# kendricktan/simple-zk-rollups

Hardware: AMD Instinct MI355X
Metric: Groth16 proofs/sec (rollup batch circuit) (higher is better)
Workload: dtype u32 limbs, 254-bit integer Montgomery (9 x 29 bits in the MSM kernels, 8 x 32 bits elsewhere); 1 GPU; 2^20-constraint synthetic rollup circuit, 1 proof per step per GPU; log_m=20, n_public=73, nVars=1048576, nnzA=1827887, nnzB=1577678, parallelism=proof-sharded x1 (key arena replicated once: single), proofs_in_flight=2

## Files before the change

include/zkr.h:

```cpp
#ifndef ZKR_H
#define ZKR_H
#include <stddef.h>
#include <stdint.h>

#ifdef __cplusplus
extern "C" {
#endif

typedef enum {
  ZKR_OK = 0,
  ZKR_ERR_NO_DEVICE = -1,
  ZKR_ERR_BAD_KEY = -2,
  ZKR_ERR_BAD_WITNESS = -3,
  ZKR_ERR_HIP = -4,
  ZKR_ERR_ARG = -5,
  ZKR_ERR_DEGENERATE = -6,
  ZKR_ERR_UNSATISFIED = -7
} zkr_status;

typedef struct zkr_key zkr_key;

const char *zkr_last_error(void);
const char *zkr_version(void);
int zkr_device_count(void);
// ... 220 lines not shown
int zkr_operator_new(zkr_ledger *l, zkr_key *key, zkr_r1cs *cs, zkr_vk *vk, const zkr_operator_opts *opts, zkr_operator **out);
void zkr_operator_free(zkr_operator *op);
int zkr_operator_info(const zkr_operator *op, uint64_t out[6]);
int zkr_operator_step(zkr_operator *op, const uint8_t *txs, size_t n_txs, const uint8_t *r32s, const uint8_t *s32s, uint8_t *status, uint8_t *proofs_out,
                      void *publics_out, size_t *n_batches, size_t *consumed);
int zkr_operator_stage_times(const zkr_operator *op, double ms[6]);

int zkr_selftest_f29_forms(int device, int field, int form, const uint32_t *records, size_t n, uint32_t *out);
int zkr_selftest_curve29(int device, int g2, int op, const uint32_t *records, size_t n, uint32_t *out, uint8_t *inf);
int zkr_selftest_fp(int device, int field, int op, const uint32_t *records, size_t n, uint32_t *out);
typedef struct {
  uint32_t logn, tlog, dif, inverse, pre, nbat, pair, in_place, want_lo, want_n, coset_shift, coset_add;
  uint32_t cross, klog, col_lo, col_n, in_sub, out_sub, canon, reserved;
} zkr_ntt_selftest_desc;
int zkr_selftest_ntt(int device, const zkr_ntt_selftest_desc *desc, void *in0, void *in1, void *out, void *in0_b, void *in1_b, void *out_b);
int zkr_bench_fq_mul(int device, double *gmuls_per_s);
int zkr_bench_fq_mul_legacy(int device, double *gmuls_per_s);

#ifdef __cplusplus
}
#endif
#endif
```

simple-zk-rollups_amd/csrc/kernels_ntt.hpp:

```cpp
#pragma once
#include <type_traits>
#include "curve.hpp"
#include "field29.hpp"

namespace zkr {

constexpr int NTT_THREADS_SMALL = 512, NTT_THREADS_LARGE = 256;
constexpr int NTT_LARGE_LOG = 21;
constexpr int NTT_TILE_LOG = 11;
constexpr int NTT_STRIDED_LOG = 9;
constexpr int NTT_W_LOG = 2;
constexpr int TWL_LOG = 10;

struct Vec32 { uint4 a, b; };

__device__ __forceinline__ Fr load_fr(const Fr *p) {
  const uint4 *q = reinterpret_cast<const uint4 *>(p);
  uint4 a = q[0], b = q[1];
  Fr r;
  r.v[0] = a.x; r.v[1] = a.y; r.v[2] = a.z; r.v[3] = a.w;
  r.v[4] = b.x; r.v[5] = b.y; r.v[6] = b.z; r.v[7] = b.w;
  return r;
}
__device__ __forceinline__ void store_fr(Fr *p, const Fr &r) {
// ... 37 lines not shown
  Fr *out_b;
  uint32_t blk_off;
  uint32_t pre_shift, pre_add;
  const Fr *x_in0[8], *x_in1[8];
  Fr *x_out[8];
  uint32_t x_in_sub, x_out_sub;
};

constexpr int NTT_H_IN = 6;
constexpr int NTT_H_DIF = 6;
constexpr int NTT_H_DIT = NTT_H_IN + 4 * NTT_TILE_LOG;
static_assert(NTT_H_DIT + 8 <= 128 && 2 * (NTT_H_DIT + 8) <= 338, "a DIT pass of NTT_TILE_LOG stages must fit the bounds of field29.hpp");
static_assert(NTT_STRIDED_LOG <= NTT_TILE_LOG, "a strided pass has no more stages than a contiguous one");
using NttL = Fr29;

template <bool DIF, bool INV, int NTT_THREADS, bool CROSS = false>
static __global__ __launch_bounds__(NTT_THREADS) void ntt_pass_kernel(const NttPassArgs a_in) {
  extern __shared__ __attribute__((aligned(16))) uint32_t lds[];
  constexpr int HL = DIF ? NTT_H_DIF : NTT_H_DIT;
  using V = L29<NttL, HL>;
  const NttPassArgs &a = a_in;
  const Fr *const in0 = blockIdx.z ? a.in0_b : a.in0, *const in1 = blockIdx.z ? a.in1_b : a.in1;
  Fr *const out = blockIdx.z ? a.out_b : a.out;
  if (a.prio == 1) __builtin_amdgcn_s_setprio(1);
  else if (a.prio == 2) __builtin_amdgcn_s_setprio(2);
  else if (a.prio == 3) __builtin_amdgcn_s_setprio(3);
  const int nb = a.hi - a.lo;
  const uint32_t rows = 1u << nb, W = 1u << a.wlog;
  const uint32_t tile = rows << a.wlog;
  const uint32_t lb = (1u << a.lo) >> a.wlog;
  const uint32_t bx = blockIdx.x + a.blk_off;
  const uint32_t q = bx / lb, l0 = (bx % lb) << a.wlog;
  const size_t base = ((size_t)blockIdx.y << a.L) + ((size_t)q << a.hi) + l0;

  auto lds_get = [&](uint32_t e) {
    V x;
#pragma unroll
    for (int k = 0; k < 9; k++) x.v[k] = lds[k * tile + e];
    return x;
  };
  auto lds_put = [&](uint32_t e, const auto &x) {
    static_assert(!DIF || std::remove_reference_t<decltype(x)>::bound <= HL, "DIF invariant broken");
#pragma unroll
    for (int k = 0; k < 9; k++) lds[k * tile + e] = x.v[k];
  };

  for (uint32_t e = threadIdx.x; e < tile; e += NTT_THREADS) {
    uint32_t r = e >> a.wlog, c = e & (W - 1);
    Fr x;
    if constexpr (CROSS) {
      const uint32_t ci = l0 + c - a.x_in_sub;
      x = load_fr(a.x_in0[r] + ci);
      if (a.pre == PRE_MUL) x = mul(x, load_fr(a.x_in1[r] + ci));
    } else {
      size_t gi = base + ((size_t)r << a.lo) + c;
      x = load_fr(in0 + gi);
      if (a.pre == PRE_COSET) {
        uint32_t br = __brev((uint32_t)gi << (32 - a.L));
        br = (br << a.pre_shift) | a.pre_add;
        x = mul(x, load_fr(a.tw + ((size_t)br << (a.tlog - a.L - a.pre_shift))));
      } else if (a.pre == PRE_MUL) {
        x = mul(x, load_fr(in1 + gi));
      }
    }
    lds_put(e, unpack29<NttL, DIF ? NTT_H_DIF : NTT_H_IN>(x.v));
  }
  __syncthreads();

  auto twiddle = [&](int slog, uint32_t x) {
    const Tw29 *tab = slog <= TWL_LOG ? a.twl29 : a.tw29;
    const int tlog = slog <= TWL_LOG ? TWL_LOG : a.tlog;
    uint32_t idx = x << (tlog - slog);
    if (INV) idx = (1u << tlog) - idx;
    return load_tw29(tab + idx);
  };
  auto dif = [&](const auto &u, const auto &v, const L29<NttL, 2> &w, auto &sum, auto &prod) {
    sum = add(u, v);
    if constexpr (INV) prod = mul(w, sub_loose(v, u)); else prod = mul(w, sub_loose(u, v));
  };
  auto dit = [&](const auto &u, const auto &v, const L29<NttL, 2> &w, auto &hi, auto &lo_) {
    auto t = mul(v, w);
    auto s = add(u, t).template to<std::remove_reference_t<decltype(hi)>::bound>();
    auto d = sub(u, t);
    if constexpr (INV) { hi = d; lo_ = s; } else { hi = s; lo_ = d; }
  };
  auto single_stage = [&](int j) {
    const uint32_t sl = 1u << j;
    for (uint32_t b = threadIdx.x; b < (tile >> 1); b += NTT_THREADS) {
      uint32_t c = b & (W - 1), kk = b >> a.wlog;
      uint32_t r0 = ((kk >> j) << (j + 1)) | (kk & (sl - 1));
      uint32_t e0 = (r0 << a.wlog) + c, e1 = e0 + (sl << a.wlog);
      auto w = twiddle(j + a.lo, ((kk & (sl - 1)) << a.lo) + l0 + c);
      V u = lds_get(e0), v = lds_get(e1);
      if constexpr (DIF) {
        L29<NttL, 2 * HL> s;
        L29<NttL, 3> p;
        dif(u, v, w, s, p);
        lds_put(e0, barrett(s));
        lds_put(e1, p);
      } else {
        L29<NttL, HL + 4> x0, x1;
        dit(u, v, w, x0, x1);
        lds_put(e0, x0);
        lds_put(e1, x1);
      }
    }
    __syncthreads();
  };
  auto double_stage = [&](int j) {
    const uint32_t sl = 1u << j;
    for (uint32_t t = threadIdx.x; t < (tile >> 2); t += NTT_THREADS) {
      uint32_t c = t & (W - 1), kq = t >> a.wlog;
      uint32_t xlow = kq & (sl - 1);
      uint32_t r00 = ((kq >> j) << (j + 2)) | xlow;
      uint32_t e00 = (r00 << a.wlog) + c, e01 = e00 + (sl << a.wlog), e10 = e00 + (sl << (a.wlog + 1)), e11 = e10 + (sl << a.wlog);
      uint32_t im = (xlow << a.lo) + l0 + c;
      auto wa = twiddle(j + a.lo, im), wb0 = twiddle(j + 1 + a.lo, im), wb1 = twiddle(j + 1 + a.lo, im + (sl << a.lo));
      V x00 = lds_get(e00), x01 = lds_get(e01), x10 = lds_get(e10), x11 = lds_get(e11);
      if constexpr (DIF) {
        L29<NttL, 2 * HL> s0, s1;
        L29<NttL, 3> p0, p1;
        dif(x00, x10, wb0, s0, p0);
        dif(x01, x11, wb1, s1, p1);
        L29<NttL, 4 * HL> ss;
        L29<NttL, 3> sp, pp;
        L29<NttL, 6> ps;
        dif(s0, s1, wa, ss, sp);
        dif(p0, p1, wa, ps, pp);
        lds_put(e00, barrett(ss));
        lds_put(e01, sp);
        lds_put(e10, ps);
        lds_put(e11, pp);
      } else {
        L29<NttL, HL + 4> y00, y01, y10, y11;
        dit(x00, x01, wa, y00, y01);
        dit(x10, x11, wa, y10, y11);
        L29<NttL, HL + 8> z00, z10, z01, z11;
        dit(y00, y10, wb0, z00, z10);
        dit(y01, y11, wb1, z01, z11);
        lds_put(e00, z00);
        lds_put(e01, z01);
        lds_put(e10, z10);
        lds_put(e11, z11);
      }
    }
    __syncthreads();
  };
  if (DIF) {
    int j = nb - 1;
    if (nb & 1) { single_stage(j); j--; }
    for (; j >= 1; j -= 2) double_stage(j - 1);
  } else {
    int j = 0;
    if (nb & 1) { single_stage(0); j = 1; }
    for (; j + 1 < nb; j += 2) double_stage(j);
  }

  for (uint32_t e = threadIdx.x; e < tile; e += NTT_THREADS) {
    uint32_t r = e >> a.wlog, c = e & (W - 1);
    V x = lds_get(e);
    Fr o;
    if constexpr (DIF) {
      static_assert(NTT_H_DIF <= NTT_H_IN, "what a DIF pass stores is what the next pass states on loading");
      if (a.canon) pack29(canonical_small(x), o.v); else pack29(x, o.v);
    } else {
      auto y = barrett(x);
      if (a.canon) pack29(canonical_small(y), o.v); else pack29(y, o.v);
    }
    if constexpr (CROSS) store_fr(a.x_out[r] + (l0 + c - a.x_out_sub), o);
    else store_fr(out + base + ((size_t)r << a.lo) + c, o);
  }
}

static __global__ void twiddle261_kernel(const Fr *T, uint32_t n, Tw29 *out) {
  uint32_t k = blockIdx.x * blockDim.x + threadIdx.x;
  if (k > n) return;
  Fr w = k < n ? load_fr(T + k) : neg(Fr::one());
// ... 124 lines not shown
```

simple-zk-rollups_amd/csrc/zkr_prove.hip:

```cpp
#include <stdio.h>
#include <stdlib.h>
#include <string.h>
#include <time.h>
#include <algorithm>
#include <memory>
#include "eval_h.hpp"
#include "kernels_msm.hpp"
#include "kernels_ntt.hpp"
#include "zkr_internal.hpp"

namespace zkr {

static const char *STAGES[] = {"ingest", "spmv", "ntt", "msm_sort", "msm_accum_g1", "msm_accum_g2", "msm_big", "msm_reduce", "total",
                               "spmv_a", "ntt_pass", "combine_h"};
static int stage_index(const char *name) {
  for (int i = 0; i < (int)(sizeof(STAGES) / sizeof(STAGES[0])); i++)
    if (!strcmp(STAGES[i], name)) return i;
  return -1;
}
static hipEvent_t next_event(ProofSlot &sl) {
  if (sl.event_next == sl.event_pool.size()) {
    ScopedEvent e;
    if (e.create()) return nullptr;
    sl.event_pool.push_back(std::move(e));
// ... 103 lines not shown
  int L;
  NttDir dir;
  int pre = PRE_NONE, nbat = 1;
  NttVecs a, b;
  uint32_t want_lo = 0, want_n = 0;
  uint32_t coset_shift = 0, coset_add = 0;
};

static NttPassArgs ntt_pass_args(const NttTables &tb, int L) {
  NttPassArgs a = {};
  a.tw = tb.tw; a.tw29 = tb.tw29; a.twl29 = tb.twl29; a.tlog = tb.tlog; a.L = L;
  a.prio = 1;
  return a;
}
template <int T, bool CROSS>
static void ntt_pass_launch_dir(NttDir dir, dim3 grid, size_t lds, hipStream_t s, const NttPassArgs &a) {
  switch (dir) {
    case DIF_INVERSE: ntt_pass_kernel<true, true, T, CROSS><<<grid, T, lds, s>>>(a); break;
    case DIF_FORWARD: ntt_pass_kernel<true, false, T, CROSS><<<grid, T, lds, s>>>(a); break;
    case DIT_FORWARD: ntt_pass_kernel<false, false, T, CROSS><<<grid, T, lds, s>>>(a); break;
    case DIT_INVERSE: ntt_pass_kernel<false, true, T, CROSS><<<grid, T, lds, s>>>(a); break;
  }
}
static void ntt_pass_launch(int threads, bool cross, NttDir dir, dim3 grid, size_t lds, hipStream_t s, const NttPassArgs &a, Prof pf) {
  const int psp = prof_begin(pf, s, "ntt_pass");
  if (cross) ntt_pass_launch_dir<NTT_THREADS_LARGE, true>(dir, grid, lds, s, a);
  else if (threads == NTT_THREADS_SMALL) ntt_pass_launch_dir<NTT_THREADS_SMALL, false>(dir, grid, lds, s, a);
  else ntt_pass_launch_dir<NTT_THREADS_LARGE, false>(dir, grid, lds, s, a);
  prof_end(pf, s, psp);
}

static int run_ntt(hipStream_t s, const NttTables &tb, const NttRun &r, Prof pf) {
  const int L = r.L;
  const bool dif = r.dir == DIF_INVERSE || r.dir == DIF_FORWARD;
  if (r.want_n && (!dif || (uint64_t)r.want_lo + r.want_n > (1ull << L))) { set_error("run_ntt: an output range needs a DIF transform and must lie inside it"); return ZKR_ERR_ARG; }
  std::vector<PassSpec> plan = ntt_plan(L, NTT_TILE_LOG);
  if (!dif) std::reverse(plan.begin(), plan.end());
  bool first = true;
  for (auto &ps : plan) {
    NttPassArgs a = ntt_pass_args(tb, L);
    a.pre_shift = r.coset_shift; a.pre_add = r.coset_add;
    a.in0 = first ? r.a.in0 : r.a.out;
    a.in1 = first ? r.a.in1 : nullptr;
    a.out = r.a.out;
    a.in0_b = first ? r.b.in0 : r.b.out;
    a.in1_b = first ? r.b.in1 : nullptr;
    a.out_b = r.b.out;
    a.lo = ps.lo; a.hi = ps.hi; a.wlog = ps.wlog;
    a.pre = first ? r.pre : PRE_NONE;
    a.canon = &ps == &plan.back() ? 1 : 0;
    uint32_t tile = 1u << (ps.hi - ps.lo + ps.wlog);
    uint32_t grid = (1u << L) / tile;
    a.blk_off = 0;
    if (r.want_n) {
      const uint32_t per_block = (1u << ps.hi) / tile;
      const uint32_t q0 = r.want_lo >> ps.hi, q1 = (uint32_t)(((uint64_t)r.want_lo + r.want_n + (1u << ps.hi) - 1) >> ps.hi);
      a.blk_off = q0 * per_block;
      grid = (q1 - q0) * per_block;
    }
    size_t lds = (size_t)tile * 36;
    const int threads = (L >= NTT_LARGE_LOG || tile <= 1024) ? NTT_THREADS_LARGE : NTT_THREADS_SMALL;
    ntt_pass_launch(threads, false, r.dir, dim3(grid, r.nbat, r.b.out ? 2 : 1), lds, s, a, pf);
    first = false;
  }
  ZKR_HIP_CHECK(hipGetLastError());
  return 0;
}

static Fr fr_from_u64(uint64_t x) {
  Fr r = Fr::zero();
  r.v[0] = (uint32_t)x;
  r.v[1] = (uint32_t)(x >> 32);
  return r;
}

static void spmv_enqueue(zkr_key *k, ProofSlot &sl, hipStream_t s, uint32_t lo, uint32_t hi, int nbat, bool with_c = false) {
  const Prof pf{k, &sl};
  const ArenaHeader &h = k->h;
  const unsigned char *ar = k->arena;
// ... 13 lines not shown
  if (with_c && ev.n_wide > nw) nw = ev.n_wide;
  if (nw) spmv_wide_kernel<<<dim3(nw, nbat, sides), 64, 0, s>>>(side[0], side[1], side[2], sl.d_w, h.m, h.n, lo, hi);
  prof_end(pf, s, sp);
}

static void combine_h_consts(uint32_t m, Fr &c1v, Fr &c2v) {
  Fr r2 = Fr::r2();
  Fr minv = inv(to_mont(fr_from_u64(m)));
  Fr half = inv(to_mont(fr_from_u64(2)));
  c1v = mul(mul(r2, half), minv);
  c2v = mul(mul(c1v, minv), minv);
}

static NttTables key_ntt_tables(const zkr_key *k) { return NttTables{(const Fr *)(k->arena + k->h.off_tw), k->tw29, k->twl29, (int)k->h.tlog}; }

static int calc_h_open(zkr_key *k, ProofSlot &sl, hipStream_t s, int nbat, int *ntt_span) {
  const Prof pf{k, &sl};
  const NttTables tb = key_ntt_tables(k);
  const int L = (int)k->h.logm;
  *ntt_span = prof_begin(pf, s, "ntt");
  if (int rc = run_ntt(s, tb, NttRun{.L = L, .dir = DIF_INVERSE, .nbat = nbat, .a = {.in0 = sl.va, .out = sl.ca}, .b = {.in0 = sl.vb, .out = sl.cb}}, pf)) return rc;
  return run_ntt(s, tb, NttRun{.L = L, .dir = DIT_FORWARD, .pre = PRE_COSET, .nbat = nbat, .a = ntt_in_place(sl.ca), .b = ntt_in_place(sl.cb)}, pf);
}

static int calc_h_device(zkr_key *k, ProofSlot &sl, hipStream_t s, int nbat) {
  const Prof pf{k, &sl};
  const ArenaHeader &h = k->h;
  const NttTables tb = key_ntt_tables(k);
  const int L = (int)h.logm;
  uint32_t m = h.m;
  spmv_enqueue(k, sl, s, 0, m, nbat);
  int sp, rc;
  const bool ranged = h.shard_parts > 1 && h.sc_n[1] < m;
  const uint32_t h_lo = ranged ? h.sc_lo[1] : 0, h_n = ranged ? h.sc_n[1] : 0;
  if ((rc = calc_h_open(k, sl, s, nbat, &sp))) return rc;
  if ((rc = run_ntt(s, tb, NttRun{.L = L, .dir = DIF_INVERSE, .pre = PRE_MUL, .nbat = nbat, .a = {.in0 = sl.ca, .in1 = sl.cb, .out = sl.ca},
                                  .b = {.in0 = sl.va, .in1 = sl.vb, .out = sl.va}, .want_lo = h_lo, .want_n = h_n}, pf))) return rc;
  Fr c1v, c2v;
  combine_h_consts(m, c1v, c2v);
  const int csp = prof_begin(pf, s, "combine_h");
  const uint32_t pos0 = ranged ? h_lo : 0, pos1 = ranged ? h_lo + h_n : m;
  combine_h_kernel<<<dim3((pos1 - pos0 + 255) / 256, nbat), 256, 0, s>>>(sl.va, sl.ca, sl.d_h, tb.tw, tb.tlog, L, c1v, c2v, sl.dig_h.rng, DIGIT_CLEAR_WORDS, pos0, pos1);
  prof_end(pf, s, csp);
  prof_end(pf, s, sp);
  ZKR_HIP_CHECK(hipGetLastError());
  return 0;
}

static int calc_h_eval(zkr_key *k, ProofSlot &sl, hipStream_t s, int nbat) {
  const Prof pf{k, &sl};
  const ArenaHeader &h = k->h;
  const uint32_t m = h.m;
  spmv_enqueue(k, sl, s, 0, m, nbat, true);
  eval_unsatisfied_kernel<<<dim3((m + 255) / 256, nbat), 256, 0, s>>>(sl.va, sl.vb, sl.d_h, m, sl.d_bad, 0, m);
  ZKR_HIP_CHECK(hipMemcpyAsync(sl.h_bad, sl.d_bad, (size_t)nbat * 4, hipMemcpyDeviceToHost, s));
  const uint32_t d0 = h.sc_lo[1], d1 = h.sc_lo[1] + h.sc_n[1];
  int sp;
  if (int rc = calc_h_open(k, sl, s, nbat, &sp)) return rc;
  const int csp = prof_begin(pf, s, "combine_h");
  eval_product_kernel<<<dim3((d1 - d0 + 255) / 256, nbat), 256, 0, s>>>(sl.ca, sl.cb, sl.d_h, m, sl.dig_h.rng, DIGIT_CLEAR_WORDS, d0, d1);
  prof_end(pf, s, csp);
  prof_end(pf, s, sp);
  ZKR_HIP_CHECK(hipGetLastError());
  return 0;
}

thread_local ShardGroup *shard_group = nullptr;
thread_local unsigned shard_group_part = 0;
thread_local bool shard_turn_held = false;

static int ntt_cross_wlog(int klog, uint32_t col_n) {
  int wlog = NTT_TILE_LOG - klog;
  while ((1u << wlog) > col_n) wlog--;
// ... 8 lines not shown
  Fr *const *rows_out;
  uint32_t in_sub = 0, out_sub = 0, col_lo, col_n;
};
static int run_ntt_cross(hipStream_t s, const NttTables &tb, const NttCross &c, Prof pf) {
  NttPassArgs a = ntt_pass_args(tb, c.L);
  a.lo = c.L - c.klog; a.hi = c.L;
  const int wlog = ntt_cross_wlog(c.klog, c.col_n);
  a.wlog = wlog;
  a.pre = c.pre;
  a.canon = c.canon ? 1 : 0;
  for (int r = 0; r < (1 << c.klog); r++) { a.x_in0[r] = c.rows_in0[r]; a.x_in1[r] = c.rows_in1 ? c.rows_in1[r] : nullptr; a.x_out[r] = c.rows_out[r]; }
  a.x_in_sub = c.in_sub; a.x_out_sub = c.out_sub;
  const uint32_t tile = 1u << (c.klog + wlog);
  a.blk_off = c.col_lo >> wlog;
  const uint32_t grid = c.col_n >> wlog;
  ntt_pass_launch(NTT_THREADS_LARGE, true, c.dir, dim3(grid), (size_t)tile * 36, s, a, pf);
  ZKR_HIP_CHECK(hipGetLastError());
  return 0;
}

static int calc_h_split(zkr_key *k, ProofSlot &sl, hipStream_t s, ShardGroup &g, unsigned part, std::unique_lock<std::mutex> &lock, bool eval) {
  struct AbortUnlessDone {
    ShardGroup &g;
    bool done = false;
    ~AbortUnlessDone() { if (!done) g.abort(); }
  } guard{g};
  const Prof pf{k, &sl};
  const ArenaHeader &h = k->h;
  const NttTables tb = key_ntt_tables(k);
  const int L = (int)h.logm, klog = g.klog, Lb = L - klog;
  const uint32_t m = h.m, P = g.parts, Bk = m >> klog, cols = Bk >> klog, col_lo = part * cols, blk = part * Bk;
// ... 942 lines not shown
    cross.in_sub = d.in_sub;
    cross.out_sub = d.out_sub;
    cross.col_lo = d.col_lo;
    cross.col_n = d.col_n;
    rc = run_ntt_cross(nullptr, tb, cross, NO_PROF);
  }
  const hipError_t e = hipDeviceSynchronize();
  if (rc) return rc;
  if (e != hipSuccess) { set_error("zkr_selftest_ntt: the run failed: %s", hipGetErrorString(e)); return ZKR_ERR_HIP; }
  int guard_bad = 0;
  for (auto &v : all)
    if ((rc = v->download(&guard_bad))) return rc;
  return guard_bad ? ZKR_ERR_HIP : 0;
}

template <class F>
static int msm_hook(const void *points_mont, const void *scalars_std, size_t n, uint8_t *out, int *is_inf, int device) {
  if (!points_mont || !scalars_std || !out || !is_inf) { set_error("null argument"); return ZKR_ERR_ARG; }
  if (int rc = need_device(device)) return rc;
  ZKR_HIP_CHECK(hipSetDevice(device));
  const size_t pb = sizeof(Affine<F>);
  const uint8_t *pts = (const uint8_t *)points_mont;
  std::vector<uint32_t> rank(n, RANK_NONE);
  uint32_t np = 0;
  std::vector<uint8_t> compact;
  for (size_t i = 0; i < n; i++) {
    bool inf = true;
    for (size_t b = 0; b < pb / 2 && inf; b++) inf = pts[i * pb + b] == 0;
    if (inf) continue;
    rank[i] = np++;
// ... 137 lines not shown
```

simple-zk-rollups_amd/python/zkr_hip/__init__.py:

```python
from .binding import (ZkrError, ProvingKey, ConstraintSystem, VerifyingKey, pairing_device, VERDICTS, lib, device_count, device_pci_bus_id, version, ntt, msm_g1, msm_g2, bench_fq_mul, selftest_f29_forms, selftest_curve29, selftest_fp, selftest_ntt, ntt_selftest_words, field_raw_ops,
                      synth_websnark, synth_witness, synth_set_shape, verify, verify_batch, contribution_check, vk_contribute, CONTRIBUTION_BYTES, ptau_new, ptau_contribute, ptau_record_check, ptau_verify, points_scale_each, points_add_each, group_ntt, PTAU_RECORD_BYTES, setup_r1cs_websnark, prove_batch_multi, prove_batch_multi_device, prove_sharded, prove_sharded_device, sharded_split_stats, sharded_last_form, sharded_last_h_form, PROOF_BYTES, PARTIAL_BYTES, STAGES)
from .facade import (build_bn128, groth16_gen_proof, proof_json_from_bytes, proof_bytes_from_json, solidity_proof, create_proof_generator,
                     binarify_verifying_key, binarify_r1cs, verifying_key_from_bytes, is_valid, cached_key, cached_replicas, cached_shards, key_fingerprint, clear_key_cache, key_cache_stats,
                     solidity_verifying_key, solidity_verifying_key_source)
from .batch import shard_indices, broadcast_key, replicate_key, broadcast_arena, prove_batch, gather_proofs

__all__ = ["ZkrError", "ProvingKey", "ConstraintSystem", "VerifyingKey", "pairing_device", "VERDICTS", "lib", "device_count", "device_pci_bus_id", "version", "ntt", "msm_g1", "msm_g2", "bench_fq_mul", "selftest_f29_forms", "selftest_curve29", "selftest_fp", "selftest_ntt", "ntt_selftest_words", "field_raw_ops",
           "synth_websnark", "synth_witness", "setup_r1cs_websnark", "cached_key", "cached_replicas", "cached_shards", "key_fingerprint", "clear_key_cache", "key_cache_stats", "solidity_verifying_key", "solidity_verifying_key_source", "synth_set_shape", "verify", "verify_batch", "contribution_check", "vk_contribute", "CONTRIBUTION_BYTES", "ptau_new", "ptau_contribute", "ptau_record_check", "ptau_verify", "points_scale_each", "points_add_each", "group_ntt", "PTAU_RECORD_BYTES", "binarify_verifying_key", "binarify_r1cs", "verifying_key_from_bytes", "is_valid", "proof_bytes_from_json", "PROOF_BYTES", "STAGES", "build_bn128", "groth16_gen_proof", "proof_json_from_bytes",
           "solidity_proof", "create_proof_generator", "prove_batch_multi", "prove_batch_multi_device", "prove_sharded", "prove_sharded_device", "sharded_split_stats", "sharded_last_form", "sharded_last_h_form", "PARTIAL_BYTES", "shard_indices", "replicate_key", "broadcast_key", "broadcast_arena", "prove_batch", "gather_proofs"]
```

simple-zk-rollups_amd/python/zkr_hip/binding.py:

```python
import ctypes
import os

_HERE = os.path.dirname(os.path.abspath(__file__))
LIB_PATH = os.environ.get("ZKR_HIP_LIB") or os.path.normpath(os.path.join(_HERE, "..", "..", "csrc", "libzkr_hip.so"))
PROOF_BYTES = 256
PARTIAL_BYTES = 640
SHARD_SIDE_TABLES = 1
CONTRIBUTION_BYTES = 352
PTAU_RECORD_BYTES = 928
REPLICATE_MODES = {"auto": 0, "full": 1, "base": 2}
KEY_SECTIONS = ("none", "rowptr", "col", "wide", "rank", "header", "points", "twiddles", "coef", "shared rank", "consts")
STAGES = ("ingest", "spmv", "ntt", "msm_sort", "msm_accum_g1", "msm_accum_g2", "msm_big", "msm_reduce", "total",
          "spmv_a", "ntt_pass", "combine_h")
_lib = None


class BookOpts(ctypes.Structure):
    _fields_ = [("nullifier_cap_log2", ctypes.c_uint32), ("reserved", ctypes.c_uint32), ("salt", ctypes.c_uint64)]


class OperatorOpts(ctypes.Structure):
    _fields_ = [("batch", ctypes.c_uint32), ("max_batches", ctypes.c_uint32), ("flags", ctypes.c_uint32), ("reserved", ctypes.c_uint32)]


# ... 102 lines not shown
    L.zkr_key_eval_tables.argtypes = [vp, u8p, sz, c.c_uint, c.POINTER(i)]
    L.zkr_key_eval_tables_drop.argtypes = [vp]
    L.zkr_key_eval_tables_equal.argtypes = [vp, vp, c.POINTER(i)]
    L.zkr_points_add_each.argtypes = [u8p, u8p, sz, i, i]
    L.zkr_setup_r1cs_websnark.argtypes = [u8p, sz, u8p, i, c.POINTER(vp), c.POINTER(sz), c.POINTER(vp), c.POINTER(sz)]
    L.zkr_synth_vk.argtypes = [vp, u8p, sz, c.POINTER(vp), c.POINTER(sz)]
    L.zkr_synth_set_shape.argtypes = [c.c_uint]
    L.zkr_free.argtypes = [vp]
    L.zkr_free.restype = None
    L.zkr_bench_fq_mul.argtypes = [i, c.POINTER(c.c_double)]
    L.zkr_bench_fq_mul_legacy.argtypes = [i, c.POINTER(c.c_double)]
    L.zkr_selftest_f29_forms.argtypes = [i, i, i, c.POINTER(c.c_uint32), sz, c.POINTER(c.c_uint32)]
    L.zkr_selftest_curve29.argtypes = [i, i, i, c.POINTER(c.c_uint32), sz, c.POINTER(c.c_uint32), c.POINTER(c.c_uint8)]
    L.zkr_selftest_fp.argtypes = [i, i, i, c.POINTER(c.c_uint32), sz, c.POINTER(c.c_uint32)]
    L.zkr_selftest_ntt.argtypes = [i, c.POINTER(NttSelftestDesc)] + [vp] * 6
    L.zkr_mimcsponge_multihash.argtypes = [u8p, sz, u8p]
    L.zkr_babyjub_pubkey.argtypes = [u8p, u8p]
    L.zkr_eddsa_sign.argtypes = [u8p, u8p, sz, u8p]
    L.zkr_eddsa_verify.argtypes = [u8p, sz, u8p, u8p, c.POINTER(i)]
    L.zkr_mimcsponge_multihash_batch.argtypes = [u8p, sz, c.c_uint, u8p, i]
    L.zkr_balance_tree_build.argtypes = [u8p, c.c_uint, u8p, i]
    L.zkr_babyjub_format_privkey.argtypes = [u8p, u8p]
    L.zkr_withdraw_r1cs.argtypes = [c.POINTER(vp), c.POINTER(sz)]
    L.zkr_withdraw_witness.argtypes = [u8p, u8p, c.POINTER(vp), c.POINTER(sz)]
    L.zkr_rollup_info.argtypes = [c.c_uint32, c.c_uint32, c.POINTER(c.c_uint32), c.POINTER(c.c_uint32), c.POINTER(c.c_uint32)]
    L.zkr_rollup_r1cs.argtypes = [c.c_uint32, c.c_uint32, c.POINTER(vp), c.POINTER(sz)]
    L.zkr_rollup_witness.argtypes = [c.c_uint32, c.c_uint32, u8p, sz, c.POINTER(vp), c.POINTER(sz)]
    L.zkr_rollup_witness_batch_device.argtypes = [c.c_uint32, c.c_uint32, u8p, sz, sz, vp, c.c_int]
    L.zkr_rollup_witness_program_host.argtypes = [c.c_uint32, c.c_uint32, u8p, sz, vp, c.POINTER(c.c_uint32), c.POINTER(c.c_uint32)]
    L.zkr_rollup_statement_text.argtypes = [c.c_uint32]
# ... 823 lines not shown
    for name, v in (("in0", in0), ("in1", in1), ("out", out), ("in0_b", in0_b), ("in1_b", in1_b), ("out_b", out_b)):
        if v is not None:
            v = bytes(v)
            bufs[name] = ctypes.create_string_buffer(v, max(1, len(v)))
    words = ntt_selftest_words(desc)
    if words is not None:
        for name, b in bufs.items():
            need = 32 * words[1 if name.startswith("out") else 0]
            if len(b) != need:
                raise ValueError("vector %s has %d bytes, the descriptor asks for %d" % (name, len(b), need))
    arg = lambda name: ctypes.cast(bufs[name], ctypes.c_void_p) if name in bufs else None
    _check(lib().zkr_selftest_ntt(device, ctypes.byref(d), arg("in0"), arg("in1"), arg("out"), arg("in0_b"), arg("in1_b"), arg("out_b")))
    return {name: b.raw for name, b in bufs.items()}


def bench_fq_mul(device=0, legacy=False) -> float:
    v = ctypes.c_double()
    _check((lib().zkr_bench_fq_mul_legacy if legacy else lib().zkr_bench_fq_mul)(device, ctypes.byref(v)))
    return v.value
```

Measured before the change: 165.2 proofs/s.

## Fuse inverse-NTT last pass with coset forward-NTT first pass in H computation

Adds a fused NTT pass mode that runs the final inverse DIF stages and the first forward DIT stages in one kernel while the data stays in LDS. It also folds the coset shift into the forward twiddles (odd-index twiddles) instead of a separate pre-multiply on load. Together these remove one global round trip of the vector and the per-element coset multiply in calc_h. The fused path is used only when nbat==1 and the pass shapes line up, and it adds new kernel template instances plus a selftest entry point.

```diff
diff --git a/include/zkr.h b/include/zkr.h
--- a/include/zkr.h
+++ b/include/zkr.h
@@ -258,6 +258,7 @@
   uint32_t cross, klog, col_lo, col_n, in_sub, out_sub, canon, reserved;
 } zkr_ntt_selftest_desc;
 int zkr_selftest_ntt(int device, const zkr_ntt_selftest_desc *desc, void *in0, void *in1, void *out, void *in0_b, void *in1_b, void *out_b);
+int zkr_selftest_ntt_eval(int device, unsigned logn, unsigned tlog, unsigned nbat, void *in_a, void *out_a, void *in_b, void *out_b);
 int zkr_bench_fq_mul(int device, double *gmuls_per_s);
 int zkr_bench_fq_mul_legacy(int device, double *gmuls_per_s);
 
diff --git a/simple-zk-rollups_amd/csrc/kernels_ntt.hpp b/simple-zk-rollups_amd/csrc/kernels_ntt.hpp
--- a/simple-zk-rollups_amd/csrc/kernels_ntt.hpp
+++ b/simple-zk-rollups_amd/csrc/kernels_ntt.hpp
@@ -75,11 +75,14 @@
 static_assert(NTT_STRIDED_LOG <= NTT_TILE_LOG, "a strided pass has no more stages than a contiguous one");
 using NttL = Fr29;
 
-template <bool DIF, bool INV, int NTT_THREADS, bool CROSS = false>
+constexpr int NTT_PLAIN = 0, NTT_COSET = 1, NTT_FUSED = 2;
+
+template <bool K_DIF, bool K_INV, int NTT_THREADS, bool CROSS = false, int MODE = NTT_PLAIN>
 static __global__ __launch_bounds__(NTT_THREADS) void ntt_pass_kernel(const NttPassArgs a_in) {
+  static_assert(MODE == NTT_PLAIN || (!K_DIF && !K_INV && !CROSS), "coset twiddles and the fused middle pass are forward DIT passes of run_ntt_eval");
   extern __shared__ __attribute__((aligned(16))) uint32_t lds[];
-  constexpr int HL = DIF ? NTT_H_DIF : NTT_H_DIT;
-  using V = L29<NttL, HL>;
+  constexpr bool FUSED = MODE == NTT_FUSED;
+  constexpr bool LOAD_DIF = K_DIF || FUSED;
   const NttPassArgs &a = a_in;
   const Fr *const in0 = blockIdx.z ? a.in0_b : a.in0, *const in1 = blockIdx.z ? a.in1_b : a.in1;
   Fr *const out = blockIdx.z ? a.out_b : a.out;
@@ -94,14 +97,13 @@
   const uint32_t q = bx / lb, l0 = (bx % lb) << a.wlog;
   const size_t base = ((size_t)blockIdx.y << a.L) + ((size_t)q << a.hi) + l0;
 
-  auto lds_get = [&](uint32_t e) {
-    V x;
+  auto lds_read = [&](auto h, uint32_t e) {
+    L29<NttL, decltype(h)::value> x;
 #pragma unroll
     for (int k = 0; k < 9; k++) x.v[k] = lds[k * tile + e];
     return x;
   };
-  auto lds_put = [&](uint32_t e, const auto &x) {
-    static_assert(!DIF || std::remove_reference_t<decltype(x)>::bound <= HL, "DIF invariant broken");
+  auto lds_write = [&](uint32_t e, const auto &x) {
 #pragma unroll
     for (int k = 0; k < 9; k++) lds[k * tile + e] = x.v[k];
   };
@@ -124,104 +126,128 @@
         x = mul(x, load_fr(in1 + gi));
       }
     }
-    lds_put(e, unpack29<NttL, DIF ? NTT_H_DIF : NTT_H_IN>(x.v));
+    lds_write(e, unpack29<NttL, LOAD_DIF ? NTT_H_DIF : NTT_H_IN>(x.v));
   }
   __syncthreads();
 
-  auto twiddle = [&](int slog, uint32_t x) {
-    const Tw29 *tab = slog <= TWL_LOG ? a.twl29 : a.tw29;
-    const int tlog = slog <= TWL_LOG ? TWL_LOG : a.tlog;
-    uint32_t idx = x << (tlog - slog);
-    if (INV) idx = (1u << tlog) - idx;
-    return load_tw29(tab + idx);
+  auto stages = [&](auto dif_c, auto inv_c, auto coset_c) {
+    constexpr bool DIF = decltype(dif_c)::value, INV = decltype(inv_c)::value, COSET = decltype(coset_c)::value;
+    constexpr int HL = DIF ? NTT_H_DIF : NTT_H_DIT;
+    using V = L29<NttL, HL>;
+    auto lds_get = [&](uint32_t e) { return lds_read(std::integral_constant<int, HL>{}, e); };
+    auto lds_put = [&](uint32_t e, const auto &x) {
+      static_assert(!DIF || std::remove_reference_t<decltype(x)>::bound <= HL, "DIF invariant broken");
+      lds_write(e, x);
+    };
+    auto twiddle = [&](int slog, uint32_t x) {
+      constexpr int top = COSET ? TWL_LOG - 1 : TWL_LOG;
+      const Tw29 *tab = slog <= top ? a.twl29 : a.tw29;
+      const int tlog = slog <= top ? TWL_LOG : a.tlog;
+      uint32_t idx;
+      if constexpr (COSET) {
+        idx = (2 * x + 1) << (tlog - slog - 1);
+      } else {
+        idx = x << (tlog - slog);
+        if (INV) idx = (1u << tlog) - idx;
+      }
+      return load_tw29(tab + idx);
+    };
+    auto dif = [&](const auto &u, const auto &v, const L29<NttL, 2> &w, auto &sum, auto &prod) {
+      sum = add(u, v);
+      if constexpr (INV) prod = mul(w, sub_loose(v, u)); else prod = mul(w, sub_loose(u, v));
+    };
+    auto dit = [&](const auto &u, const auto &v, const L29<NttL, 2> &w, auto &hi, auto &lo_) {
+      auto t = mul(v, w);
+      auto s = add(u, t).template to<std::remove_reference_t<decltype(hi)>::bound>();
+      auto d = sub(u, t);
+      if constexpr (INV) { hi = d; lo_ = s; } else { hi = s; lo_ = d; }
+    };
+    auto single_stage = [&](int j) {
+      const uint32_t sl = 1u << j;
+      for (uint32_t b = threadIdx.x; b < (tile >> 1); b += NTT_THREADS) {
+        uint32_t c = b & (W - 1), kk = b >> a.wlog;
+        uint32_t r0 = ((kk >> j) << (j + 1)) | (kk & (sl - 1));
+        uint32_t e0 = (r0 << a.wlog) + c, e1 = e0 + (sl << a.wlog);
+        auto w = twiddle(j + a.lo, ((kk & (sl - 1)) << a.lo) + l0 + c);
+        V u = lds_get(e0), v = lds_get(e1);
+        if constexpr (DIF) {
+          L29<NttL, 2 * HL> s;
+          L29<NttL, 3> p;
+          dif(u, v, w, s, p);
+          lds_put(e0, barrett(s));
+          lds_put(e1, p);
+        } else {
+          L29<NttL, HL + 4> x0, x1;
+          dit(u, v, w, x0, x1);
+          lds_put(e0, x0);
+          lds_put(e1, x1);
+        }
+      }
+      __syncthreads();
+    };
+    auto double_stage = [&](int j) {
+      const uint32_t sl = 1u << j;
+      for (uint32_t t = threadIdx.x; t < (tile >> 2); t += NTT_THREADS) {
+        uint32_t c = t & (W - 1), kq = t >> a.wlog;
+        uint32_t xlow = kq & (sl - 1);
+        uint32_t r00 = ((kq >> j) << (j + 2)) | xlow;
+        uint32_t e00 = (r00 << a.wlog) + c, e01 = e00 + (sl << a.wlog), e10 = e00 + (sl << (a.wlog + 1)), e11 = e10 + (sl << a.wlog);
+        uint32_t im = (xlow << a.lo) + l0 + c;
+        auto wa = twiddle(j + a.lo, im), wb0 = twiddle(j + 1 + a.lo, im), wb1 = twiddle(j + 1 + a.lo, im + (sl << a.lo));
+        V x00 = lds_get(e00), x01 = lds_get(e01), x10 = lds_get(e10), x11 = lds_get(e11);
+        if constexpr (DIF) {
+          L29<NttL, 2 * HL> s0, s1;
+          L29<NttL, 3> p0, p1;
+          dif(x00, x10, wb0, s0, p0);
+          dif(x01, x11, wb1, s1, p1);
+          L29<NttL, 4 * HL> ss;
+          L29<NttL, 3> sp, pp;
+          L29<NttL, 6> ps;
+          dif(s0, s1, wa, ss, sp);
+          dif(p0, p1, wa, ps, pp);
+          lds_put(e00, barrett(ss));
+          lds_put(e01, sp);
+          lds_put(e10, ps);
+          lds_put(e11, pp);
+        } else {
+          L29<NttL, HL + 4> y00, y01, y10, y11;
+          dit(x00, x01, wa, y00, y01);
+          dit(x10, x11, wa, y10, y11);
+          L29<NttL, HL + 8> z00, z10, z01, z11;
+          dit(y00, y10, wb0, z00, z10);
+          dit(y01, y11, wb1, z01, z11);
+          lds_put(e00, z00);
+          lds_put(e01, z01);
+          lds_put(e10, z10);
+          lds_put(e11, z11);
+        }
+      }
+      __syncthreads();
+    };
+    if (DIF) {
+      int j = nb - 1;
+      if (nb & 1) { single_stage(j); j--; }
+      for (; j >= 1; j -= 2) double_stage(j - 1);
+    } else {
+      int j = 0;
+      if (nb & 1) { single_stage(0); j = 1; }
+      for (; j + 1 < nb; j += 2) double_stage(j);
+    }
   };
-  auto dif = [&](const auto &u, const auto &v, const L29<NttL, 2> &w, auto &sum, auto &prod) {
-    sum = add(u, v);
-    if constexpr (INV) prod = mul(w, sub_loose(v, u)); else prod = mul(w, sub_loose(u, v));
-  };
-  auto dit = [&](const auto &u, const auto &v, const L29<NttL, 2> &w, auto &hi, auto &lo_) {
-    auto t = mul(v, w);
-    auto s = add(u, t).template to<std::remove_reference_t<decltype(hi)>::bound>();
-    auto d = sub(u, t);
-    if constexpr (INV) { hi = d; lo_ = s; } else { hi = s; lo_ = d; }
-  };
-  auto single_stage = [&](int j) {
-    const uint32_t sl = 1u << j;
-    for (uint32_t b = threadIdx.x; b < (tile >> 1); b += NTT_THREADS) {
-      uint32_t c = b & (W - 1), kk = b >> a.wlog;
-      uint32_t r0 = ((kk >> j) << (j + 1)) | (kk & (sl - 1));
-      uint32_t e0 = (r0 << a.wlog) + c, e1 = e0 + (sl << a.wlog);
-      auto w = twiddle(j + a.lo, ((kk & (sl - 1)) << a.lo) + l0 + c);
-      V u = lds_get(e0), v = lds_get(e1);
-      if constexpr (DIF) {
-        L29<NttL, 2 * HL> s;
-        L29<NttL, 3> p;
-        dif(u, v, w, s, p);
-        lds_put(e0, barrett(s));
-        lds_put(e1, p);
-      } else {
-        L29<NttL, HL + 4> x0, x1;
-        dit(u, v, w, x0, x1);
-        lds_put(e0, x0);
-        lds_put(e1, x1);
-      }
-    }
-    __syncthreads();
-  };
-  auto double_stage = [&](int j) {
-    const uint32_t sl = 1u << j;
-    for (uint32_t t = threadIdx.x; t < (tile >> 2); t += NTT_THREADS) {
-      uint32_t c = t & (W - 1), kq = t >> a.wlog;
-      uint32_t xlow = kq & (sl - 1);
-      uint32_t r00 = ((kq >> j) << (j + 2)) | xlow;
-      uint32_t e00 = (r00 << a.wlog) + c, e01 = e00 + (sl << a.wlog), e10 = e00 + (sl << (a.wlog + 1)), e11 = e10 + (sl << a.wlog);
-      uint32_t im = (xlow << a.lo) + l0 + c;
-      auto wa = twiddle(j + a.lo, im), wb0 = twiddle(j + 1 + a.lo, im), wb1 = twiddle(j + 1 + a.lo, im + (sl << a.lo));
-      V x00 = lds_get(e00), x01 = lds_get(e01), x10 = lds_get(e10), x11 = lds_get(e11);
-      if constexpr (DIF) {
-        L29<NttL, 2 * HL> s0, s1;
-        L29<NttL, 3> p0, p1;
-        dif(x00, x10, wb0, s0, p0);
-        dif(x01, x11, wb1, s1, p1);
-        L29<NttL, 4 * HL> ss;
-        L29<NttL, 3> sp, pp;
-        L29<NttL, 6> ps;
-        dif(s0, s1, wa, ss, sp);
-        dif(p0, p1, wa, ps, pp);
-        lds_put(e00, barrett(ss));
-        lds_put(e01, sp);
-        lds_put(e10, ps);
-        lds_put(e11, pp);
-      } else {
-        L29<NttL, HL + 4> y00, y01, y10, y11;
-        dit(x00, x01, wa, y00, y01);
-        dit(x10, x11, wa, y10, y11);
-        L29<NttL, HL + 8> z00, z10, z01, z11;
-        dit(y00, y10, wb0, z00, z10);
-        dit(y01, y11, wb1, z01, z11);
-        lds_put(e00, z00);
-        lds_put(e01, z01);
-        lds_put(e10, z10);
-        lds_put(e11, z11);
-      }
-    }
-    __syncthreads();
-  };
-  if (DIF) {
-    int j = nb - 1;
-    if (nb & 1) { single_stage(j); j--; }
-    for (; j >= 1; j -= 2) double_stage(j - 1);
+  using std::bool_constant;
+  if constexpr (FUSED) {
+    static_assert(NTT_H_DIF <= NTT_H_IN, "a fused pass hands DIF outputs to DIT stages inside LDS");
+    stages(bool_constant<true>{}, bool_constant<true>{}, bool_constant<false>{});
+    stages(bool_constant<false>{}, bool_constant<false>{}, bool_constant<true>{});
   } else {
-    int j = 0;
-    if (nb & 1) { single_stage(0); j = 1; }
-    for (; j + 1 < nb; j += 2) double_stage(j);
+    stages(bool_constant<K_DIF>{}, bool_constant<K_INV>{}, bool_constant<MODE == NTT_COSET>{});
   }
 
   for (uint32_t e = threadIdx.x; e < tile; e += NTT_THREADS) {
     uint32_t r = e >> a.wlog, c = e & (W - 1);
-    V x = lds_get(e);
+    auto x = lds_read(std::integral_constant<int, K_DIF ? NTT_H_DIF : NTT_H_DIT>{}, e);
     Fr o;
-    if constexpr (DIF) {
+    if constexpr (K_DIF) {
       static_assert(NTT_H_DIF <= NTT_H_IN, "what a DIF pass stores is what the next pass states on loading");
       if (a.canon) pack29(canonical_small(x), o.v); else pack29(x, o.v);
     } else {
diff --git a/simple-zk-rollups_amd/csrc/zkr_prove.hip b/simple-zk-rollups_amd/csrc/zkr_prove.hip
--- a/simple-zk-rollups_amd/csrc/zkr_prove.hip
+++ b/simple-zk-rollups_amd/csrc/zkr_prove.hip
@@ -141,7 +141,11 @@
   return a;
 }
 template <int T, bool CROSS>
-static void ntt_pass_launch_dir(NttDir dir, dim3 grid, size_t lds, hipStream_t s, const NttPassArgs &a) {
+static void ntt_pass_launch_dir(NttDir dir, int mode, dim3 grid, size_t lds, hipStream_t s, const NttPassArgs &a) {
+  if constexpr (!CROSS) {
+    if (mode == NTT_COSET) { ntt_pass_kernel<false, false, T, false, NTT_COSET><<<grid, T, lds, s>>>(a); return; }
+    if (mode == NTT_FUSED) { ntt_pass_kernel<false, false, T, false, NTT_FUSED><<<grid, T, lds, s>>>(a); return; }
+  }
   switch (dir) {
     case DIF_INVERSE: ntt_pass_kernel<true, true, T, CROSS><<<grid, T, lds, s>>>(a); break;
     case DIF_FORWARD: ntt_pass_kernel<true, false, T, CROSS><<<grid, T, lds, s>>>(a); break;
@@ -149,12 +153,39 @@
     case DIT_INVERSE: ntt_pass_kernel<false, true, T, CROSS><<<grid, T, lds, s>>>(a); break;
   }
 }
-static void ntt_pass_launch(int threads, bool cross, NttDir dir, dim3 grid, size_t lds, hipStream_t s, const NttPassArgs &a, Prof pf) {
+static void ntt_pass_launch(int threads, bool cross, NttDir dir, int mode, dim3 grid, size_t lds, hipStream_t s, const NttPassArgs &a, Prof pf) {
   const int psp = prof_begin(pf, s, "ntt_pass");
-  if (cross) ntt_pass_launch_dir<NTT_THREADS_LARGE, true>(dir, grid, lds, s, a);
-  else if (threads == NTT_THREADS_SMALL) ntt_pass_launch_dir<NTT_THREADS_SMALL, false>(dir, grid, lds, s, a);
-  else ntt_pass_launch_dir<NTT_THREADS_LARGE, false>(dir, grid, lds, s, a);
+  if (cross) ntt_pass_launch_dir<NTT_THREADS_LARGE, true>(dir, NTT_PLAIN, grid, lds, s, a);
+  else if (threads == NTT_THREADS_SMALL) ntt_pass_launch_dir<NTT_THREADS_SMALL, false>(dir, mode, grid, lds, s, a);
+  else ntt_pass_launch_dir<NTT_THREADS_LARGE, false>(dir, mode, grid, lds, s, a);
   prof_end(pf, s, psp);
+}
+
+static void ntt_run_pass(hipStream_t s, const NttTables &tb, const NttRun &r, const PassSpec &ps, bool first, bool last, NttDir dir, int mode, Prof pf) {
+  const int L = r.L;
+  NttPassArgs a = ntt_pass_args(tb, L);
+  a.pre_shift = r.coset_shift; a.pre_add = r.coset_add;
+  a.in0 = first ? r.a.in0 : r.a.out;
+  a.in1 = first ? r.a.in1 : nullptr;
+  a.out = r.a.out;
+  a.in0_b = first ? r.b.in0 : r.b.out;
+  a.in1_b = first ? r.b.in1 : nullptr;
+  a.out_b = r.b.out;
+  a.lo = ps.lo; a.hi = ps.hi; a.wlog = ps.wlog;
+  a.pre = first ? r.pre : PRE_NONE;
+  a.canon = last ? 1 : 0;
+  uint32_t tile = 1u << (ps.hi - ps.lo + ps.wlog);
+  uint32_t grid = (1u << L) / tile;
+  a.blk_off = 0;
+  if (r.want_n) {
+    const uint32_t per_block = (1u << ps.hi) / tile;
+    const uint32_t q0 = r.want_lo >> ps.hi, q1 = (uint32_t)(((uint64_t)r.want_lo + r.want_n + (1u << ps.hi) - 1) >> ps.hi);
+    a.blk_off = q0 * per_block;
+    grid = (q1 - q0) * per_block;
+  }
+  size_t lds = (size_t)tile * 36;
+  const int threads = (L >= NTT_LARGE_LOG || tile <= 1024) ? NTT_THREADS_LARGE : NTT_THREADS_SMALL;
+  ntt_pass_launch(threads, false, dir, mode, dim3(grid, r.nbat, r.b.out ? 2 : 1), lds, s, a, pf);
 }
 
 static int run_ntt(hipStream_t s, const NttTables &tb, const NttRun &r, Prof pf) {
@@ -163,33 +194,26 @@
   if (r.want_n && (!dif || (uint64_t)r.want_lo + r.want_n > (1ull << L))) { set_error("run_ntt: an output range needs a DIF transform and must lie inside it"); return ZKR_ERR_ARG; }
   std::vector<PassSpec> plan = ntt_plan(L, NTT_TILE_LOG);
   if (!dif) std::reverse(plan.begin(), plan.end());
-  bool first = true;
-  for (auto &ps : plan) {
-    NttPassArgs a = ntt_pass_args(tb, L);
-    a.pre_shift = r.coset_shift; a.pre_add = r.coset_add;
-    a.in0 = first ? r.a.in0 : r.a.out;
-    a.in1 = first ? r.a.in1 : nullptr;
-    a.out = r.a.out;
-    a.in0_b = first ? r.b.in0 : r.b.out;
-    a.in1_b = first ? r.b.in1 : nullptr;
-    a.out_b = r.b.out;
-    a.lo = ps.lo; a.hi = ps.hi; a.wlog = ps.wlog;
-    a.pre = first ? r.pre : PRE_NONE;
-    a.canon = &ps == &plan.back() ? 1 : 0;
-    uint32_t tile = 1u << (ps.hi - ps.lo + ps.wlog);
-    uint32_t grid = (1u << L) / tile;
-    a.blk_off = 0;
-    if (r.want_n) {
-      const uint32_t per_block = (1u << ps.hi) / tile;
-      const uint32_t q0 = r.want_lo >> ps.hi, q1 = (uint32_t)(((uint64_t)r.want_lo + r.want_n + (1u << ps.hi) - 1) >> ps.hi);
-      a.blk_off = q0 * per_block;
-      grid = (q1 - q0) * per_block;
-    }
-    size_t lds = (size_t)tile * 36;
-    const int threads = (L >= NTT_LARGE_LOG || tile <= 1024) ? NTT_THREADS_LARGE : NTT_THREADS_SMALL;
-    ntt_pass_launch(threads, false, r.dir, dim3(grid, r.nbat, r.b.out ? 2 : 1), lds, s, a, pf);
-    first = false;
-  }
+  for (auto &ps : plan) ntt_run_pass(s, tb, r, ps, &ps == &plan.front(), &ps == &plan.back(), r.dir, NTT_PLAIN, pf);
+  ZKR_HIP_CHECK(hipGetLastError());
+  return 0;
+}
+
+static int run_ntt_eval(hipStream_t s, const NttTables &tb, int L, int nbat, const NttVecs &a, const NttVecs &b, bool fuse, Prof pf) {
+  if (tb.tlog < L) { set_error("run_ntt_eval: the twiddle table must cover the transform"); return ZKR_ERR_ARG; }
+  const std::vector<PassSpec> inv = ntt_plan(L, NTT_TILE_LOG);
+  std::vector<PassSpec> fwd = inv;
+  std::reverse(fwd.begin(), fwd.end());
+  const PassSpec &il = inv.back(), &ff = fwd.front();
+  if (!fuse || !(il.lo == 0 && ff.lo == 0 && il.hi == ff.hi && il.wlog == 0 && ff.wlog == 0)) {
+    if (int rc = run_ntt(s, tb, NttRun{.L = L, .dir = DIF_INVERSE, .nbat = nbat, .a = a, .b = b}, pf)) return rc;
+    return run_ntt(s, tb, NttRun{.L = L, .dir = DIT_FORWARD, .pre = PRE_COSET, .nbat = nbat, .a = ntt_in_place(a.out), .b = b.out ? ntt_in_place(b.out) : NttVecs{}}, pf);
+  }
+  const NttRun r{.L = L, .dir = DIT_FORWARD, .nbat = nbat, .a = a, .b = b};
+  const size_t ni = inv.size(), nf = fwd.size();
+  for (size_t i = 0; i + 1 < ni; i++) ntt_run_pass(s, tb, r, inv[i], i == 0, false, DIF_INVERSE, NTT_PLAIN, pf);
+  ntt_run_pass(s, tb, r, ff, ni == 1, nf == 1, DIT_FORWARD, NTT_FUSED, pf);
+  for (size_t i = 1; i < nf; i++) ntt_run_pass(s, tb, r, fwd[i], false, i + 1 == nf, DIT_FORWARD, NTT_COSET, pf);
   ZKR_HIP_CHECK(hipGetLastError());
   return 0;
 }
@@ -233,15 +257,6 @@
 
 static NttTables key_ntt_tables(const zkr_key *k) { return NttTables{(const Fr *)(k->arena + k->h.off_tw), k->tw29, k->twl29, (int)k->h.tlog}; }
 
-static int calc_h_open(zkr_key *k, ProofSlot &sl, hipStream_t s, int nbat, int *ntt_span) {
-  const Prof pf{k, &sl};
-  const NttTables tb = key_ntt_tables(k);
-  const int L = (int)k->h.logm;
-  *ntt_span = prof_begin(pf, s, "ntt");
-  if (int rc = run_ntt(s, tb, NttRun{.L = L, .dir = DIF_INVERSE, .nbat = nbat, .a = {.in0 = sl.va, .out = sl.ca}, .b = {.in0 = sl.vb, .out = sl.cb}}, pf)) return rc;
-  return run_ntt(s, tb, NttRun{.L = L, .dir = DIT_FORWARD, .pre = PRE_COSET, .nbat = nbat, .a = ntt_in_place(sl.ca), .b = ntt_in_place(sl.cb)}, pf);
-}
-
 static int calc_h_device(zkr_key *k, ProofSlot &sl, hipStream_t s, int nbat) {
   const Prof pf{k, &sl};
   const ArenaHeader &h = k->h;
@@ -249,10 +264,12 @@
   const int L = (int)h.logm;
   uint32_t m = h.m;
   spmv_enqueue(k, sl, s, 0, m, nbat);
-  int sp, rc;
+  int rc;
   const bool ranged = h.shard_parts > 1 && h.sc_n[1] < m;
   const uint32_t h_lo = ranged ? h.sc_lo[1] : 0, h_n = ranged ? h.sc_n[1] : 0;
-  if ((rc = calc_h_open(k, sl, s, nbat, &sp))) return rc;
+  const int sp = prof_begin(pf, s, "ntt");
+  if ((rc = run_ntt(s, tb, NttRun{.L = L, .dir = DIF_INVERSE, .nbat = nbat, .a = {.in0 = sl.va, .out = sl.ca}, .b = {.in0 = sl.vb, .out = sl.cb}}, pf))) return rc;
+  if ((rc = run_ntt(s, tb, NttRun{.L = L, .dir = DIT_FORWARD, .pre = PRE_COSET, .nbat = nbat, .a = ntt_in_place(sl.ca), .b = ntt_in_place(sl.cb)}, pf))) return rc;
   if ((rc = run_ntt(s, tb, NttRun{.L = L, .dir = DIF_INVERSE, .pre = PRE_MUL, .nbat = nbat, .a = {.in0 = sl.ca, .in1 = sl.cb, .out = sl.ca},
                                   .b = {.in0 = sl.va, .in1 = sl.vb, .out = sl.va}, .want_lo = h_lo, .want_n = h_n}, pf))) return rc;
   Fr c1v, c2v;
@@ -274,8 +291,8 @@
   eval_unsatisfied_kernel<<<dim3((m + 255) / 256, nbat), 256, 0, s>>>(sl.va, sl.vb, sl.d_h, m, sl.d_bad, 0, m);
   ZKR_HIP_CHECK(hipMemcpyAsync(sl.h_bad, sl.d_bad, (size_t)nbat * 4, hipMemcpyDeviceToHost, s));
   const uint32_t d0 = h.sc_lo[1], d1 = h.sc_lo[1] + h.sc_n[1];
-  int sp;
-  if (int rc = calc_h_open(k, sl, s, nbat, &sp)) return rc;
+  const int sp = prof_begin(pf, s, "ntt");
+  if (int rc = run_ntt_eval(s, key_ntt_tables(k), (int)h.logm, nbat, NttVecs{.in0 = sl.va, .out = sl.ca}, NttVecs{.in0 = sl.vb, .out = sl.cb}, nbat == 1, pf)) return rc;
   const int csp = prof_begin(pf, s, "combine_h");
   eval_product_kernel<<<dim3((d1 - d0 + 255) / 256, nbat), 256, 0, s>>>(sl.ca, sl.cb, sl.d_h, m, sl.dig_h.rng, DIGIT_CLEAR_WORDS, d0, d1);
   prof_end(pf, s, csp);
@@ -314,7 +331,7 @@
   const uint32_t tile = 1u << (c.klog + wlog);
   a.blk_off = c.col_lo >> wlog;
   const uint32_t grid = c.col_n >> wlog;
-  ntt_pass_launch(NTT_THREADS_LARGE, true, c.dir, dim3(grid), (size_t)tile * 36, s, a, pf);
+  ntt_pass_launch(NTT_THREADS_LARGE, true, c.dir, NTT_PLAIN, dim3(grid), (size_t)tile * 36, s, a, pf);
   ZKR_HIP_CHECK(hipGetLastError());
   return 0;
 }
@@ -1287,6 +1304,35 @@
   return guard_bad ? ZKR_ERR_HIP : 0;
 }
 
+extern "C" int zkr_selftest_ntt_eval(int device, unsigned logn, unsigned tlog, unsigned nbat, void *in_a, void *out_a, void *in_b, void *out_b) {
+  auto bad = [](const char *what) { set_error("zkr_selftest_ntt_eval: %s", what); return ZKR_ERR_ARG; };
+  if (logn < 1 || logn > 22) return bad("logn must be 1 .. 22");
+  if (tlog < logn || tlog > 24) return bad("tlog must be logn .. 24");
+  if (nbat < 1 || ((uint64_t)nbat << logn) > (1ull << 24)) return bad("nbat must be at least 1, with nbat 2^logn at most 2^24 elements");
+  if (!in_a || !out_a) return bad("null vector (in_a, out_a)");
+  if (!in_b != !out_b) return bad("the second transform takes in_b and out_b, or neither");
+  if (int rc = need_device(device)) return rc;
+  ZKR_HIP_CHECK(hipSetDevice(device));
+  if (int lrc = ntt_lds_check(device)) return lrc;
+  HookNttTables tables;
+  int rc;
+  if ((rc = tables.build(tlog))) return rc;
+  const size_t n = (size_t)nbat << logn;
+  NttTestVec va, oa, vb, ob;
+  if ((rc = va.upload("in_a", 0, in_a, n, true)) || (rc = oa.upload("out_a", 0, out_a, n, false))) return rc;
+  if (in_b && ((rc = vb.upload("in_b", 0, in_b, n, true)) || (rc = ob.upload("out_b", 0, out_b, n, false)))) return rc;
+  ZKR_HIP_CHECK(hipGetLastError());
+  rc = run_ntt_eval(nullptr, tables.view(), (int)logn, (int)nbat, NttVecs{.in0 = va.data(), .out = oa.data()},
+                    in_b ? NttVecs{.in0 = vb.data(), .out = ob.data()} : NttVecs{}, true, NO_PROF);
+  const hipError_t e = hipDeviceSynchronize();
+  if (rc) return rc;
+  if (e != hipSuccess) { set_error("zkr_selftest_ntt_eval: the run failed: %s", hipGetErrorString(e)); return ZKR_ERR_HIP; }
+  int guard_bad = 0;
+  for (NttTestVec *v : {&va, &oa, &vb, &ob})
+    if (v->host && (rc = v->download(&guard_bad))) return rc;
+  return guard_bad ? ZKR_ERR_HIP : 0;
+}
+
 template <class F>
 static int msm_hook(const void *points_mont, const void *scalars_std, size_t n, uint8_t *out, int *is_inf, int device) {
   if (!points_mont || !scalars_std || !out || !is_inf) { set_error("null argument"); return ZKR_ERR_ARG; }
diff --git a/simple-zk-rollups_amd/python/zkr_hip/__init__.py b/simple-zk-rollups_amd/python/zkr_hip/__init__.py
--- a/simple-zk-rollups_amd/python/zkr_hip/__init__.py
+++ b/simple-zk-rollups_amd/python/zkr_hip/__init__.py
@@ -1,10 +1,10 @@
-from .binding import (ZkrError, ProvingKey, ConstraintSystem, VerifyingKey, pairing_device, VERDICTS, lib, device_count, device_pci_bus_id, version, ntt, msm_g1, msm_g2, bench_fq_mul, selftest_f29_forms, selftest_curve29, selftest_fp, selftest_ntt, ntt_selftest_words, field_raw_ops,
+from .binding import (ZkrError, ProvingKey, ConstraintSystem, VerifyingKey, pairing_device, VERDICTS, lib, device_count, device_pci_bus_id, version, ntt, msm_g1, msm_g2, bench_fq_mul, selftest_f29_forms, selftest_curve29, selftest_fp, selftest_ntt, selftest_ntt_eval, ntt_selftest_words, field_raw_ops,
                       synth_websnark, synth_witness, synth_set_shape, verify, verify_batch, contribution_check, vk_contribute, CONTRIBUTION_BYTES, ptau_new, ptau_contribute, ptau_record_check, ptau_verify, points_scale_each, points_add_each, group_ntt, PTAU_RECORD_BYTES, setup_r1cs_websnark, prove_batch_multi, prove_batch_multi_device, prove_sharded, prove_sharded_device, sharded_split_stats, sharded_last_form, sharded_last_h_form, PROOF_BYTES, PARTIAL_BYTES, STAGES)
 from .facade import (build_bn128, groth16_gen_proof, proof_json_from_bytes, proof_bytes_from_json, solidity_proof, create_proof_generator,
                      binarify_verifying_key, binarify_r1cs, verifying_key_from_bytes, is_valid, cached_key, cached_replicas, cached_shards, key_fingerprint, clear_key_cache, key_cache_stats,
                      solidity_verifying_key, solidity_verifying_key_source)
 from .batch import shard_indices, broadcast_key, replicate_key, broadcast_arena, prove_batch, gather_proofs
 
-__all__ = ["ZkrError", "ProvingKey", "ConstraintSystem", "VerifyingKey", "pairing_device", "VERDICTS", "lib", "device_count", "device_pci_bus_id", "version", "ntt", "msm_g1", "msm_g2", "bench_fq_mul", "selftest_f29_forms", "selftest_curve29", "selftest_fp", "selftest_ntt", "ntt_selftest_words", "field_raw_ops",
+__all__ = ["ZkrError", "ProvingKey", "ConstraintSystem", "VerifyingKey", "pairing_device", "VERDICTS", "lib", "device_count", "device_pci_bus_id", "version", "ntt", "msm_g1", "msm_g2", "bench_fq_mul", "selftest_f29_forms", "selftest_curve29", "selftest_fp", "selftest_ntt", "selftest_ntt_eval", "ntt_selftest_words", "field_raw_ops",
            "synth_websnark", "synth_witness", "setup_r1cs_websnark", "cached_key", "cached_replicas", "cached_shards", "key_fingerprint", "clear_key_cache", "key_cache_stats", "solidity_verifying_key", "solidity_verifying_key_source", "synth_set_shape", "verify", "verify_batch", "contribution_check", "vk_contribute", "CONTRIBUTION_BYTES", "ptau_new", "ptau_contribute", "ptau_record_check", "ptau_verify", "points_scale_each", "points_add_each", "group_ntt", "PTAU_RECORD_BYTES", "binarify_verifying_key", "binarify_r1cs", "verifying_key_from_bytes", "is_valid", "proof_bytes_from_json", "PROOF_BYTES", "STAGES", "build_bn128", "groth16_gen_proof", "proof_json_from_bytes",
            "solidity_proof", "create_proof_generator", "prove_batch_multi", "prove_batch_multi_device", "prove_sharded", "prove_sharded_device", "sharded_split_stats", "sharded_last_form", "sharded_last_h_form", "PARTIAL_BYTES", "shard_indices", "replicate_key", "broadcast_key", "broadcast_arena", "prove_batch", "gather_proofs"]
diff --git a/simple-zk-rollups_amd/python/zkr_hip/binding.py b/simple-zk-rollups_amd/python/zkr_hip/binding.py
--- a/simple-zk-rollups_amd/python/zkr_hip/binding.py
+++ b/simple-zk-rollups_amd/python/zkr_hip/binding.py
@@ -140,6 +140,7 @@
     L.zkr_selftest_curve29.argtypes = [i, i, i, c.POINTER(c.c_uint32), sz, c.POINTER(c.c_uint32), c.POINTER(c.c_uint8)]
     L.zkr_selftest_fp.argtypes = [i, i, i, c.POINTER(c.c_uint32), sz, c.POINTER(c.c_uint32)]
     L.zkr_selftest_ntt.argtypes = [i, c.POINTER(NttSelftestDesc)] + [vp] * 6
+    L.zkr_selftest_ntt_eval.argtypes = [i, c.c_uint, c.c_uint, c.c_uint] + [vp] * 4
     L.zkr_mimcsponge_multihash.argtypes = [u8p, sz, u8p]
     L.zkr_babyjub_pubkey.argtypes = [u8p, u8p]
     L.zkr_eddsa_sign.argtypes = [u8p, u8p, sz, u8p]
@@ -993,6 +994,20 @@
     return {name: b.raw for name, b in bufs.items()}
 
 
+def selftest_ntt_eval(logn, in_a, in_b=None, nbat=1, tlog=None, fill=0xA5, device=0):
+    n = 32 * (int(nbat) << int(logn))
+    bufs = {"in_a": bytes(in_a), "out_a": bytes([fill]) * n}
+    if in_b is not None:
+        bufs.update(in_b=bytes(in_b), out_b=bytes([fill]) * n)
+    for name, v in bufs.items():
+        if len(v) != n:
+            raise ValueError("vector %s has %d bytes, nbat 2^logn words are %d" % (name, len(v), n))
+    bufs = {name: ctypes.create_string_buffer(v, len(v)) for name, v in bufs.items()}
+    arg = lambda name: ctypes.cast(bufs[name], ctypes.c_void_p) if name in bufs else None
+    _check(lib().zkr_selftest_ntt_eval(device, int(logn), int(logn if tlog is None else tlog), int(nbat), arg("in_a"), arg("out_a"), arg("in_b"), arg("out_b")))
+    return {name: b.raw for name, b in bufs.items()}
+
+
 def bench_fq_mul(device=0, legacy=False) -> float:
     v = ctypes.c_double()
     _check((lib().zkr_bench_fq_mul_legacy if legacy else lib().zkr_bench_fq_mul)(device, ctypes.byref(v)))
```

After: 165.4 proofs/s, median of 4. Within noise of the previous version (+0.1%).
